# themattinthehatt/behavenet

Hardware: AMD Instinct MI355X
Metric: AE training frames/sec (128x128x1, batch 256) (higher is better)
Workload: dtype f32; 1 GPU; configs[1]: conv AE default arch, 1x128x128 f32 frames resident in HBM, 12 latents, batch 256 (chunks 200+56), fwd+bwd+Adam(amsgrad)

## Files before the change

behavenet_amd/csrc/conv_qgemm.hip:

```cpp
#include <stdlib.h>
#include "bn_common.h"
#include "bn_fast.h"

typedef float floatx16 __attribute__((ext_vector_type(16)));

#define QG_T 64
#define QG_NB 2
#define QG_KS 32
#define QG_LD 33
enum { QG_DOWN = 0, QG_UP = 1, QG_WGRAD = 2 };

struct QGArgs {
    const float* small;
    const float* big;
    const float* w;
    float* part;
    int N, Cs, Cb;
    int M, Nc, K;
    int kper;
    float* out;
    const float* bias;
    const float* dact_src;
    int act, dact;
    float slope;
};

__device__ __forceinline__ int qg_pix(int z, int j) {
    return (4 * (z >> 1) + (j >> 2)) * 8 + 4 * (z & 1) + (j & 3);
}
__device__ __forceinline__ int qg_tap(int z, int j) {
    return (((z >> 1) ? 0 : 1) + (j >> 2)) * 5 + ((z & 1) ? 0 : 1) + (j & 3);
}

typedef float floatx4a __attribute__((ext_vector_type(4)));
typedef float floatx4u __attribute__((ext_vector_type(4), aligned(4)));

template <int MODE>
__global__ __launch_bounds__(256) void k_qgemm(QGArgs a) {
    __shared__ float As[QG_T * QG_LD];
    __shared__ float Bs[QG_NB * QG_T * QG_LD];
    const int tid = threadIdx.x, lane = tid & 63;
    const int wv = __builtin_amdgcn_readfirstlane(tid >> 6);
    const int li = lane & 31, lk = lane >> 5;
    const int z = blockIdx.z & 3, ks = blockIdx.z >> 2;
    const int i0 = blockIdx.y * QG_T, j0 = blockIdx.x * (QG_NB * QG_T);
    const int kbeg = ks * a.kper;
    const int kend = min(a.K, kbeg + a.kper);
    const int zp = z >> 1, zq = z & 1;

    int ar, ak, br, bk;
    if (MODE == QG_WGRAD) { ar = tid & 63; ak = (tid >> 6) * 8; }
    else                  { ar = tid >> 2; ak = (tid & 3) * 8; }
    if (MODE == QG_DOWN)  { br = tid >> 2; bk = (tid & 3) * 8; }
    else                  { bk = tid >> 3; br = (tid & 7) * 8; }
    const bool a_ok = (i0 + ar) < a.M;

    constexpr int OOB = 0x7fffffff;
    const void* a_base = (MODE == QG_DOWN) ? (const void*)a.big : (const void*)a.small;
    const size_t a_bytes = (MODE == QG_DOWN) ? (size_t)a.N * a.Cb * 64 * 4 : (size_t)a.N * a.Cs * 4 * 4;
    const void* b_base = (MODE == QG_WGRAD) ? (const void*)a.big : (const void*)a.w;
    const size_t b_bytes = (MODE == QG_WGRAD) ? (size_t)a.N * a.Cb * 64 * 4 : (size_t)a.Cs * a.Cb * 25 * 4;
    const __amdgpu_buffer_rsrc_t rsa = __builtin_amdgcn_make_buffer_rsrc((void*)a_base, 0, (int)a_bytes, 0x00020000);
    const __amdgpu_buffer_rsrc_t rsb = __builtin_amdgcn_make_buffer_rsrc((void*)b_base, 0, (int)b_bytes, 0x00020000);
    int avo, bvo[QG_NB], a_step, b_step, a_e = 0;
    if (MODE == QG_DOWN) {
        avo = (((i0 + ar) * a.Cb + (ak >> 4)) * 64 + (4 * zp + ((ak & 15) >> 2)) * 8 + 4 * zq) * 4;
        a_step = 2 * 64 * 4;
    } else if (MODE == QG_UP) {
        avo = (z * a.N * a.Cs + (i0 + ar) * a.Cs + ak) * 4;
        a_step = QG_KS * 4;
    } else {
        avo = ((ak * a.Cs + i0 + ar) * 4 + z) * 4;
        a_e = a.Cs * 16;
        a_step = QG_KS * a.Cs * 16;
    }
    if (!a_ok) avo = OOB;
#pragma unroll
    for (int h = 0; h < QG_NB; ++h) {
        const int jc = j0 + QG_T * h + br;
        if (MODE == QG_DOWN)
            bvo[h] = ((jc * a.Cb + (bk >> 4)) * 25 + ((zp ? 0 : 1) + ((bk & 15) >> 2)) * 5 + (zq ? 0 : 1)) * 4;
        else if (MODE == QG_UP)
            bvo[h] = ((bk * a.Cb + (jc >> 4)) * 25 + ((zp ? 0 : 1) + ((jc & 15) >> 2)) * 5 + (zq ? 0 : 1)) * 4;
        else
            bvo[h] = ((bk * a.Cb + (jc >> 4)) * 64 + (4 * zp + ((jc & 15) >> 2)) * 8 + 4 * zq) * 4;
    }
    b_step = (MODE == QG_DOWN) ? 2 * 25 * 4 : (MODE == QG_UP ? QG_KS * a.Cb * 25 * 4 : QG_KS * a.Cb * 64 * 4);
    constexpr int B2ND = (MODE == QG_WGRAD) ? 32 : 20;

    float ra[8], rb[QG_NB][8];
    auto fetch = [&](const int sidx, const int k0) __attribute__((always_inline)) {
        const int sa = (MODE == QG_DOWN ? (kbeg >> 4) * 256 : (MODE == QG_UP ? kbeg * 4 : kbeg * a.Cs * 16)) + sidx * a_step;
        const int sb = (MODE == QG_DOWN ? (kbeg >> 4) * 100 : (MODE == QG_UP ? kbeg * a.Cb * 100 : kbeg * a.Cb * 256)) + sidx * b_step;
        const bool tail = (MODE == QG_WGRAD) && (k0 + QG_KS > kend);
        if (MODE == QG_WGRAD) {
#pragma unroll
            for (int e = 0; e < 8; ++e) {
                const int vo = (tail && k0 + ak + e >= kend) ? OOB : avo;
                ra[e] = __builtin_bit_cast(float, __builtin_amdgcn_raw_buffer_load_b32(rsa, vo, sa + e * a_e, 0));
            }
        } else {
            const floatx4a v0 = __builtin_bit_cast(floatx4a, __builtin_amdgcn_raw_buffer_load_b128(rsa, avo, sa, 0));
            const floatx4a v1 = __builtin_bit_cast(floatx4a, __builtin_amdgcn_raw_buffer_load_b128(
                rsa, avo, sa + (MODE == QG_DOWN ? 32 : 16), 0));
            ra[0] = v0.x; ra[1] = v0.y; ra[2] = v0.z; ra[3] = v0.w;
            ra[4] = v1.x; ra[5] = v1.y; ra[6] = v1.z; ra[7] = v1.w;
        }
#pragma unroll
        for (int h = 0; h < QG_NB; ++h) {
            const int vo = (tail && k0 + bk >= kend) ? OOB : bvo[h];
            const floatx4a w0 = __builtin_bit_cast(floatx4a, __builtin_amdgcn_raw_buffer_load_b128(rsb, vo, sb, 0));
            const floatx4a w1 = __builtin_bit_cast(floatx4a, __builtin_amdgcn_raw_buffer_load_b128(rsb, vo, sb + B2ND, 0));
            rb[h][0] = w0.x; rb[h][1] = w0.y; rb[h][2] = w0.z; rb[h][3] = w0.w;
            rb[h][4] = w1.x; rb[h][5] = w1.y; rb[h][6] = w1.z; rb[h][7] = w1.w;
        }
    };

    floatx16 acc[QG_NB];
#pragma unroll
    for (int h = 0; h < QG_NB; ++h)
#pragma unroll
        for (int t = 0; t < 16; ++t) acc[h][t] = 0.f;
    const float* ap = As + ((wv >> 1) * 32 + li) * QG_LD + lk;
    const float* bp = Bs + ((wv & 1) * 32 + li) * QG_LD + lk;

    if (kbeg < kend) fetch(0, kbeg);
    int sidx = 0;
#ifdef QG_LOOP_SHIFT
    BN_LOOP_PLACE(8, QG_LOOP_SHIFT);
#endif
    for (int k0 = kbeg; k0 < kend; k0 += QG_KS, ++sidx) {
        __syncthreads();
#pragma unroll
        for (int e = 0; e < 8; ++e) As[ar * QG_LD + ak + e] = ra[e];
#pragma unroll
        for (int h = 0; h < QG_NB; ++h)
#pragma unroll
            for (int e = 0; e < 8; ++e) {
                if (MODE == QG_DOWN) Bs[(QG_T * h + br) * QG_LD + bk + e] = rb[h][e];
                else                 Bs[(QG_T * h + br + e) * QG_LD + bk] = rb[h][e];
            }
        __syncthreads();
#pragma unroll
        for (int t = 0; t < QG_KS / 2; ++t) {
            const float av = ap[2 * t];
#pragma unroll
            for (int h = 0; h < QG_NB; ++h)
                acc[h] = __builtin_amdgcn_mfma_f32_32x32x2f32(av, bp[QG_T * h * QG_LD + 2 * t],
                                                              acc[h], 0, 0, 0);
            if (t == 1) {
                __builtin_amdgcn_sched_barrier(0);
                if (k0 + QG_KS < kend) fetch(sidx + 1, k0 + QG_KS);
                __builtin_amdgcn_sched_barrier(0);
            }
        }
    }

    if (MODE == QG_UP) {
        const int obytes = (int)((size_t)a.M * a.Cb * 64 * 4);
        const __amdgpu_buffer_rsrc_t ro = __builtin_amdgcn_make_buffer_rsrc((void*)a.out, 0, obytes, 0x00020000);
        const __amdgpu_buffer_rsrc_t rd = __builtin_amdgcn_make_buffer_rsrc(
            (void*)a.dact_src, 0, a.dact_src ? obytes : 0, 0x00020000);
        const int row_bytes = a.Cb * 64 * 4;
        const int irow = i0 + (wv >> 1) * 32 + 4 * lk;
        if (a.act != BN_ACT_SIGMOID && a.dact != BN_ACT_SIGMOID) {
            const float es = (a.act == BN_ACT_LRELU) ? a.slope : 1.f;
            const float ds = (a.dact == BN_ACT_LRELU) ? a.slope : 1.f;
#pragma unroll
            for (int h = 0; h < QG_NB; ++h) {
                const int j = j0 + QG_T * h + (wv & 1) * 32 + li;
                const int c = j >> 4;
                const float bj = a.bias ? a.bias[c] : 0.f;
                const int vo = (irow * a.Cb * 64 + c * 64 + qg_pix(z, j & 15)) * 4;
                float d[16];
                if (a.dact_src) {
#pragma unroll
                    for (int t = 0; t < 16; ++t) {
                        const int ro_t = (t & 3) + 8 * (t >> 2);
                        d[t] = __builtin_bit_cast(float, __builtin_amdgcn_raw_buffer_load_b32(
                            rd, (irow + ro_t < a.M) ? vo : 0x7fffffff, ro_t * row_bytes, 0));
                    }
                }
#pragma unroll
                for (int t = 0; t < 16; ++t) {
                    const int ro_t = (t & 3) + 8 * (t >> 2);
                    float v = acc[h][t] + bj;
                    v = v > 0.f ? v : v * es;
                    if (a.dact_src) v *= d[t] > 0.f ? 1.f : ds;
                    __builtin_amdgcn_raw_buffer_store_b32(__builtin_bit_cast(int, v), ro,
                                                          (irow + ro_t < a.M) ? vo : 0x7fffffff,
                                                          ro_t * row_bytes, 0);
                }
            }
            return;
        }
#pragma unroll
        for (int h = 0; h < QG_NB; ++h) {
            const int j = j0 + QG_T * h + (wv & 1) * 32 + li;
            const int c = j >> 4;
            const float bj = a.bias ? a.bias[c] : 0.f;
            const size_t col = (size_t)c * 64 + qg_pix(z, j & 15);
#pragma unroll
            for (int t = 0; t < 16; ++t) {
                const int i = i0 + (wv >> 1) * 32 + (t & 3) + 8 * (t >> 2) + 4 * lk;
                if (i >= a.M) continue;
                const size_t o = (size_t)i * a.Cb * 64 + col;
                float v = bn_apply_act(acc[h][t] + bj, a.act, a.slope);
                if (a.dact_src) v *= bn_act_grad_from_output(a.dact_src[o], a.dact, a.slope);
                a.out[o] = v;
            }
        }
        return;
    }
    float* dst = a.part + ((size_t)(ks * 4 + z) * a.M) * a.Nc;
#pragma unroll
    for (int h = 0; h < QG_NB; ++h) {
        const int j = j0 + QG_T * h + (wv & 1) * 32 + li;
#pragma unroll
        for (int t = 0; t < 16; ++t) {
            const int i = i0 + (wv >> 1) * 32 + (t & 3) + 8 * (t >> 2) + 4 * lk;
            if (i < a.M) dst[(size_t)i * a.Nc + j] = acc[h][t];
        }
    }
}

__global__ __launch_bounds__(256) void k_qg_split_small(const float* __restrict__ small,
                                                        float* __restrict__ dst, size_t nm) {
    const size_t idx = (size_t)blockIdx.x * 256 + threadIdx.x;
    if (idx >= nm) return;
    const floatx4a v = *reinterpret_cast<const floatx4a*>(small + 4 * idx);
    dst[idx] = v.x; dst[nm + idx] = v.y; dst[2 * nm + idx] = v.z; dst[3 * nm + idx] = v.w;
}

__global__ __launch_bounds__(256) void k_qg_finish_down(
    const float* __restrict__ part, const float* __restrict__ bias, float* __restrict__ out,
    const float* __restrict__ dact_src, int N, int Cs, int splits, int act, int dact,
    float slope) {
    const size_t total = (size_t)N * Cs * 4;
    const size_t idx = (size_t)blockIdx.x * 256 + threadIdx.x;
    if (idx >= total) return;
    const int z = (int)(idx & 3);
    const size_t nm = idx >> 2;
    const size_t plane = (size_t)N * Cs;
    float v = 0.f;
    for (int s = 0; s < splits; ++s) v += part[(size_t)(s * 4 + z) * plane + nm];
    if (bias) v += bias[nm % Cs];
    v = bn_apply_act(v, act, slope);
    if (dact_src) v *= bn_act_grad_from_output(dact_src[idx], dact, slope);
    out[idx] = v;
}

__global__ __launch_bounds__(256) void k_qg_finish_wgrad(
    const float* __restrict__ part, float* __restrict__ dw, int Cs, int Cb, int accumulate) {
    __shared__ __attribute__((aligned(16))) float stage[256 * 25];
    const size_t npair = (size_t)Cs * Cb;
    const size_t mc = (size_t)blockIdx.x * 256 + threadIdx.x;
    const size_t plane = npair * 16;
    if (mc < npair) {
        float q[4][16];
#pragma unroll
        for (int zq = 0; zq < 4; ++zq)
#pragma unroll
            for (int g4 = 0; g4 < 4; ++g4) {
                const floatx4a v = *reinterpret_cast<const floatx4a*>(part + zq * plane + mc * 16 + 4 * g4);
                q[zq][4 * g4 + 0] = v.x; q[zq][4 * g4 + 1] = v.y; q[zq][4 * g4 + 2] = v.z; q[zq][4 * g4 + 3] = v.w;
            }
#pragma unroll
        for (int tap = 0; tap < 25; ++tap) {
            const int r = tap / 5, s = tap - 5 * r;
            float v = 0.f;
#pragma unroll
            for (int p = 0; p < 2; ++p) {
                const int yy = r - (p ? 0 : 1);
                if (yy < 0 || yy > 3) continue;
#pragma unroll
                for (int qq = 0; qq < 2; ++qq) {
                    const int xx = s - (qq ? 0 : 1);
                    if (xx < 0 || xx > 3) continue;
                    v += q[2 * p + qq][4 * yy + xx];
                }
            }
            stage[threadIdx.x * 25 + tap] = v;
        }
    }
    __syncthreads();
    const size_t base = (size_t)blockIdx.x * 256 * 25;
    const size_t total = npair * 25;
    for (int i = threadIdx.x; i < 256 * 25 / 4; i += 256) {
        const size_t o = base + 4 * (size_t)i;
        if (o + 3 < total) {
            floatx4a v = *reinterpret_cast<const floatx4a*>(stage + 4 * i);
            if (accumulate) {
                const floatx4a d = *reinterpret_cast<const floatx4a*>(dw + o);
                v.x += d.x; v.y += d.y; v.z += d.z; v.w += d.w;
            }
            *reinterpret_cast<floatx4a*>(dw + o) = v;
        } else {
            for (int e = 0; e < 4; ++e)
                if (o + e < total) dw[o + e] = accumulate ? dw[o + e] + stage[4 * i + e] : stage[4 * i + e];
        }
    }
}

bool bn_qgemm_supported(const BnGeom& g) {
    if (g.R != 5 || g.S != 5 || g.stride != 5) return false;
    if (g.Hs != 2 || g.Ws != 2 || g.Hb != 8 || g.Wb != 8 || g.pt != 1 || g.pl != 1) return false;
    if ((g.Cs % (QG_NB * QG_T)) != 0 || (g.Cb % (4 * QG_NB)) != 0) return false;
    if ((size_t)g.N * g.Cb * 64 * 4 >= 0x7fffffffull) return false;
    return true;
}

static int qg_down_splits(const BnGeom& g) {
    if ((g.Cs / QG_T) * 4 >= 64) return 1;
    int s = g.Cb * 16 >= 4096 ? 4 : (g.Cb * 16 >= 2048 ? 2 : 1);
    if (g.N <= 64) {
        const int tiles = (g.Cs / (QG_NB * QG_T)) * ((g.N + QG_T - 1) / QG_T) * 4;
        while (tiles * s < 256 && s < 16 && (g.Cb * 16) / (2 * s) >= 256) s *= 2;
    }
    return s;
}

size_t bn_qgemm_ws_bytes(int role, const BnGeom& g) {
    if (role == QG_DOWN) return (size_t)qg_down_splits(g) * 4 * g.N * g.Cs * sizeof(float);
    if (role == QG_UP) return (size_t)4 * g.N * g.Cs * sizeof(float);
    return (size_t)4 * g.Cs * g.Cb * 16 * sizeof(float);
}

int bn_launch_qgemm_down(const float* big, const float* w, const float* bias, float* out,
                         const float* dact_src, const BnGeom& g, int act, int dact, float slope,
                         void* ws, hipStream_t st) {
    const int splits = qg_down_splits(g);
    QGArgs a = {nullptr, big, w, (float*)ws, g.N, g.Cs, g.Cb, g.N, g.Cs, g.Cb * 16, 0,
                nullptr, nullptr, nullptr, 0, 0, 0.f};
    a.kper = ((a.K / splits + QG_KS - 1) / QG_KS) * QG_KS;
    const dim3 grid(a.Nc / (QG_NB * QG_T), (a.M + QG_T - 1) / QG_T, 4 * splits);
    BN_LAUNCH_MAIN(k_qgemm<QG_DOWN>, grid, dim3(256), 0, st, a);
    BN_LAUNCH_CHECK();
    const size_t total = (size_t)g.N * g.Cs * 4;
    hipLaunchKernelGGL(k_qg_finish_down, dim3((unsigned)((total + 255) / 256)), dim3(256), 0, st,
                       (const float*)ws, bias, out, dact_src, g.N, g.Cs, splits, act, dact, slope);
    BN_LAUNCH_CHECK();
    return 0;
}

int bn_launch_qgemm_up(const float* small, const float* w, const float* bias, float* out,
                       const float* dact_src, const BnGeom& g, int act, int dact, float slope,
                       void* ws, hipStream_t st) {
    float* zsmall = (float*)ws;
    const size_t nm = (size_t)g.N * g.Cs;
    hipLaunchKernelGGL(k_qg_split_small, dim3((unsigned)((nm + 255) / 256)), dim3(256), 0, st, small,
                       zsmall, nm);
    BN_LAUNCH_CHECK();
    QGArgs a = {zsmall, nullptr, w, nullptr, g.N, g.Cs, g.Cb, g.N, g.Cb * 16, g.Cs, 0,
                out, bias, dact_src, act, dact, slope};
    a.kper = ((a.K + QG_KS - 1) / QG_KS) * QG_KS;
    const dim3 grid(a.Nc / (QG_NB * QG_T), (a.M + QG_T - 1) / QG_T, 4);
    BN_LAUNCH_MAIN(k_qgemm<QG_UP>, grid, dim3(256), 0, st, a);
    BN_LAUNCH_CHECK();
    return 0;
}

int bn_launch_qgemm_wgrad(const float* small, const float* big, float* dw, const BnGeom& g,
                          int accumulate, void* ws, hipStream_t st) {
    QGArgs a = {small, big, nullptr, (float*)ws, g.N, g.Cs, g.Cb, g.Cs, g.Cb * 16, g.N, 0,
                nullptr, nullptr, nullptr, 0, 0, 0.f};
    a.kper = ((a.K + QG_KS - 1) / QG_KS) * QG_KS;
    const dim3 grid(a.Nc / (QG_NB * QG_T), (a.M + QG_T - 1) / QG_T, 4);
    BN_LAUNCH_MAIN(k_qgemm<QG_WGRAD>, grid, dim3(256), 0, st, a);
    BN_LAUNCH_CHECK();
    const size_t npair = (size_t)g.Cs * g.Cb;
    hipLaunchKernelGGL(k_qg_finish_wgrad, dim3((unsigned)((npair + 255) / 256)), dim3(256), 0, st,
                       (const float*)ws, dw, g.Cs, g.Cb, accumulate);
    BN_LAUNCH_CHECK();
    return 0;
}
```

behavenet_amd/csrc/conv_qgemm2.hip:

```cpp
#include <stdlib.h>
#include "bn_common.h"
#include "bn_fast.h"

typedef float q2x16 __attribute__((ext_vector_type(16)));
typedef float q2x4 __attribute__((ext_vector_type(4)));

#define Q2_THREADS 256
#define Q2_OOB 0x7fffffff
#define Q2_MAX_LDS (160 * 1024)

__device__ __forceinline__ void q2_dma16(__amdgpu_buffer_rsrc_t rsrc, char* lds, int voffset,
                                         int soffset) {
    __builtin_amdgcn_raw_ptr_buffer_load_lds(rsrc, (float*)lds, 16, voffset, soffset, 0, 0);
}

#define Q2_R0(z) (((z) >> 1) ? 0 : 1)
#define Q2_S0(z) (((z) & 1) ? 0 : 1)

#define Q2U_KS 32
#define Q2U_PAIR 1040
#define Q2U_SBYTES (16 * Q2U_PAIR)
#define Q2U_WROW 200
#define Q2U_WINSTR 25
#define Q2U_WBYTES (Q2U_WINSTR * 1024)
#define Q2U_STAGE (Q2U_SBYTES + Q2U_WBYTES)
#define Q2U_NDMA 11

__global__ __launch_bounds__(Q2_THREADS, 1) void k_qg2_up(
    const float* __restrict__ small, const float* __restrict__ w, const float* __restrict__ bias,
    float* __restrict__ out, const float* __restrict__ dact_src, int N, int Cs, int Cb, int act,
    int dact, float slope) {
    extern __shared__ __attribute__((aligned(16))) char smem[];
    const int tid = threadIdx.x, lane = tid & 63;
    const int wv = __builtin_amdgcn_readfirstlane(tid >> 6);
    const int li = lane & 31, kh = lane >> 5;
    const int cw0 = blockIdx.x * 8, c0 = cw0 + 2 * wv, n0 = blockIdx.y * 32;

    const __amdgpu_buffer_rsrc_t rs_s = __builtin_amdgcn_make_buffer_rsrc(
        (void*)small, 0, (int)((size_t)N * Cs * 16), 0x00020000);
    const __amdgpu_buffer_rsrc_t rs_w = __builtin_amdgcn_make_buffer_rsrc(
        (void*)w, 0, (int)((size_t)Cs * Cb * 100), 0x00020000);

    const int vo_s = ((n0 + (lane >> 5)) * Cs + (lane & 31)) * 16;
    int vo_w[7];
#pragma unroll
    for (int h = 0; h < 7; ++h) {
        const int grp = 64 * (wv + 4 * h) + lane;
        const int ml = grp / 50, gi = grp - 50 * ml;
        vo_w[h] = (ml * Cb + cw0) * 100 + gi * 16;
    }
    auto issue_dma = [&](const int d, const int buf, const int stage) __attribute__((always_inline)) {
        char* base = smem + buf * Q2U_STAGE;
        if (d < 4) {
            q2_dma16(rs_s, base + (4 * wv + d) * Q2U_PAIR, vo_s, (2 * (4 * wv + d) * Cs + stage * Q2U_KS) * 16);
        } else {
            const int h = d - 4;
            if (wv + 4 * h < Q2U_WINSTR)
                q2_dma16(rs_w, base + Q2U_SBYTES + (wv + 4 * h) * 1024, vo_w[h], stage * Q2U_KS * Cb * 100);
        }
    };

    const int ad_s = (li >> 1) * Q2U_PAIR + ((li & 1) * 32 + kh) * 16;
    const int jj = li & 15;
    const int ad_w = Q2U_SBYTES + (kh * Q2U_WROW + (2 * wv + (li >> 4)) * 25 + (jj >> 2) * 5 + (jj & 3)) * 4;

    q2x16 acc[4];
#pragma unroll
    for (int z = 0; z < 4; ++z)
#pragma unroll
        for (int t = 0; t < 16; ++t) acc[z][t] = 0.f;

    const int n_stages = Cs / Q2U_KS;
#pragma unroll
    for (int d = 0; d < Q2U_NDMA; ++d) issue_dma(d, 0, 0);

#ifdef Q2U_LOOP_SHIFT
    BN_LOOP_PLACE(8, Q2U_LOOP_SHIFT);
#endif
    for (int st = 0; st < n_stages; ++st) {
        asm volatile("s_waitcnt vmcnt(0)" ::: "memory");
        __syncthreads();
        const int buf = st & 1;
#ifdef Q2_ABL_NODMA
        const bool more = false;
#else
        const bool more = st + 1 < n_stages;
#endif
        const char* sp = smem + buf * Q2U_STAGE + ad_s;
        int wo[4];
#pragma unroll
        for (int z = 0; z < 4; ++z) {
            wo[z] = buf * Q2U_STAGE + ad_w + (Q2_R0(z) * 5 + Q2_S0(z)) * 4;
            asm volatile("" : "+v"(wo[z]));
        }
        q2x4 sv[2];
        float wq[2][4];
        sv[0] = *reinterpret_cast<const q2x4*>(sp);
#pragma unroll
        for (int z = 0; z < 4; ++z) wq[0][z] = *reinterpret_cast<const float*>(smem + wo[z]);
#pragma unroll
        for (int t = 0; t < 16; ++t) {
            const int cu = t & 1, nx = cu ^ 1;
            if (t + 1 < 16) {
                sv[nx] = *reinterpret_cast<const q2x4*>(sp + (t + 1) * 32);
#pragma unroll
                for (int z = 0; z < 4; ++z)
                    wq[nx][z] = *reinterpret_cast<const float*>(smem + wo[z] + (t + 1) * 2 * Q2U_WROW * 4);
            }
            __builtin_amdgcn_sched_barrier(0);
            acc[0] = __builtin_amdgcn_mfma_f32_32x32x2f32(wq[cu][0], sv[cu].x, acc[0], 0, 0, 0);
            acc[1] = __builtin_amdgcn_mfma_f32_32x32x2f32(wq[cu][1], sv[cu].y, acc[1], 0, 0, 0);
            if (more && t < Q2U_NDMA) issue_dma(t, buf ^ 1, st + 1);
            acc[2] = __builtin_amdgcn_mfma_f32_32x32x2f32(wq[cu][2], sv[cu].z, acc[2], 0, 0, 0);
            acc[3] = __builtin_amdgcn_mfma_f32_32x32x2f32(wq[cu][3], sv[cu].w, acc[3], 0, 0, 0);
            __builtin_amdgcn_sched_barrier(0);
        }
    }

    const int n = n0 + li;
    const int obytes = (int)((size_t)N * Cb * 64 * 4);
    const __amdgpu_buffer_rsrc_t ro = __builtin_amdgcn_make_buffer_rsrc((void*)out, 0, obytes, 0x00020000);
    const __amdgpu_buffer_rsrc_t rd = __builtin_amdgcn_make_buffer_rsrc(
        (void*)dact_src, 0, dact_src ? obytes : 0, 0x00020000);
    const int vo = (n < N) ? (n * Cb + c0) * 256 : Q2_OOB;
    const float es = (act == BN_ACT_LRELU) ? slope : 1.f;
    const float ds = (dact == BN_ACT_LRELU) ? slope : 1.f;
    float bz[2] = {0.f, 0.f};
    if (bias) { bz[0] = bias[c0]; bz[1] = bias[c0 + 1]; }
#pragma unroll
    for (int z = 0; z < 4; ++z) {
        q2x4 d[4];
#pragma unroll
        for (int tq = 0; tq < 4; ++tq) {
            const int so = (tq >> 1) * 256 + ((4 * (z >> 1) + 2 * (tq & 1)) * 8 + 4 * (z & 1)) * 4;
            if (dact_src)
                d[tq] = __builtin_bit_cast(q2x4, __builtin_amdgcn_raw_buffer_load_b128(rd, vo + kh * 32, so, 0));
        }
#pragma unroll
        for (int tq = 0; tq < 4; ++tq) {
            const int so = (tq >> 1) * 256 + ((4 * (z >> 1) + 2 * (tq & 1)) * 8 + 4 * (z & 1)) * 4;
            q2x4 v;
#pragma unroll
            for (int e = 0; e < 4; ++e) {
                float x = acc[z][4 * tq + e] + bz[tq >> 1];
                x = x > 0.f ? x : x * es;
                if (dact_src) x *= d[tq][e] > 0.f ? 1.f : ds;
                v[e] = x;
            }
            __builtin_amdgcn_raw_buffer_store_b128(__builtin_bit_cast(__attribute__((ext_vector_type(4))) unsigned int, v),
                                                   ro, vo + kh * 32, so, 0);
        }
    }
}

bool bn_qg2_up_supported(const BnGeom& g, int act, int dact) {
    if (!bn_qgemm_supported(g)) return false;
    if (act == BN_ACT_SIGMOID || dact == BN_ACT_SIGMOID) return false;
    if ((g.Cs % Q2U_KS) != 0 || (g.Cb & 7) != 0) return false;
    if (((g.N + 31) / 32) * (g.Cb / 8) < 128) return false;
    return true;
}

int bn_launch_qg2_up(const float* small, const float* w, const float* bias, float* out,
                     const float* dact_src, const BnGeom& g, int act, int dact, float slope,
                     hipStream_t st) {
    static bool attr_set = false;
    if (!attr_set) {
        hipError_t e = hipFuncSetAttribute((const void*)k_qg2_up, hipFuncAttributeMaxDynamicSharedMemorySize,
                                           Q2_MAX_LDS);
        if (e != hipSuccess) return (int)e;
        attr_set = true;
    }
    const dim3 grid(g.Cb / 8, (g.N + 31) / 32);
    BN_LAUNCH_MAIN(k_qg2_up, grid, dim3(Q2_THREADS), (size_t)2 * Q2U_STAGE, st, small, w, bias, out,
                   dact_src, g.N, g.Cs, g.Cb, act, dact, slope);
    BN_LAUNCH_CHECK();
    return 0;
}

#define Q2W_KS 16
#define Q2W_SBYTES (Q2W_KS * 1024)
#define Q2W_BBYTES (Q2W_KS * 2048)
#define Q2W_STAGE (Q2W_SBYTES + Q2W_BBYTES)
#define Q2W_NBUF 3
#define Q2W_NDMA 12

__global__ __launch_bounds__(Q2_THREADS, 1) void k_qg2_wgrad(
    const float* __restrict__ small, const float* __restrict__ big, float* __restrict__ dw,
    float* __restrict__ db, int N, int Cs, int Cb, int accumulate, int bias_side) {
    extern __shared__ __attribute__((aligned(16))) char smem[];
    const int tid = threadIdx.x, lane = tid & 63;
    const int wv = __builtin_amdgcn_readfirstlane(tid >> 6);
    const int li = lane & 31, kh = lane >> 5;
    const int mb = wv & 1, cq = wv >> 1;
    const int c0 = blockIdx.x * 8, m0 = blockIdx.y * 64;

    const __amdgpu_buffer_rsrc_t rs_s = __builtin_amdgcn_make_buffer_rsrc(
        (void*)small, 0, (int)((size_t)N * Cs * 16), 0x00020000);
    const __amdgpu_buffer_rsrc_t rs_b = __builtin_amdgcn_make_buffer_rsrc(
        (void*)big, 0, (int)((size_t)N * Cb * 256), 0x00020000);
    const int vo_s = (m0 + lane) * 16;
    const int vo_b = c0 * 256 + lane * 16;
    auto issue_dma = [&](const int d, const int buf, const int stage) __attribute__((always_inline)) {
        char* base = smem + buf * Q2W_STAGE;
        if (d < 4) {
            const int nl = 4 * wv + d;
            q2_dma16(rs_s, base + nl * 1024, vo_s, (stage * Q2W_KS + nl) * Cs * 16);
        } else {
            const int nl = 4 * wv + ((d - 4) >> 1), half = (d - 4) & 1;
            q2_dma16(rs_b, base + Q2W_SBYTES + nl * 2048 + half * 1024, vo_b,
                     (stage * Q2W_KS + nl) * Cb * 256 + half * 1024);
        }
    };

    const int jj = li & 15;
    const int ad_a = (kh * 64 + 32 * mb + li) * 16;
    const int ad_b = Q2W_SBYTES + (kh * 512 + (4 * cq + (li >> 4)) * 64 + (jj >> 2) * 8 + (jj & 3)) * 4;

    q2x16 acc[2][4];
#pragma unroll
    for (int cb = 0; cb < 2; ++cb)
#pragma unroll
        for (int z = 0; z < 4; ++z)
#pragma unroll
            for (int t = 0; t < 16; ++t) acc[cb][z][t] = 0.f;
    float bsum = 0.f;
    const bool do_bias1 = (bias_side == 1) && db && blockIdx.x == 0;
    const bool do_bias2 = (bias_side == 2) && db && blockIdx.y == 0;

    const int n_stages = (N + Q2W_KS - 1) / Q2W_KS;
#pragma unroll
    for (int d = 0; d < Q2W_NDMA; ++d) issue_dma(d, 0, 0);
    if (n_stages > 1) {
#pragma unroll
        for (int d = 0; d < Q2W_NDMA; ++d) issue_dma(d, 1, 1);
    }

    int buf = 0;
#ifdef Q2W_LOOP_SHIFT
    BN_LOOP_PLACE(8, Q2W_LOOP_SHIFT);
#endif
    for (int st = 0; st < n_stages; ++st) {
        if (st + 1 < n_stages) asm volatile("s_waitcnt vmcnt(12)" ::: "memory");
        else                   asm volatile("s_waitcnt vmcnt(0)" ::: "memory");
        __builtin_amdgcn_s_barrier();
        const bool more = st + 2 < n_stages;
        const int nbuf = (buf + 2 >= Q2W_NBUF) ? buf + 2 - Q2W_NBUF : buf + 2;
        const char* base = smem + buf * Q2W_STAGE;
        if (do_bias1) {
            const char* p = base + ((tid >> 6) * 4 * 64 + (tid & 63)) * 16;
#pragma unroll
            for (int i = 0; i < 4; ++i) {
                const q2x4 v = *reinterpret_cast<const q2x4*>(p + i * 1024);
                bsum += (v.x + v.y) + (v.z + v.w);
            }
        }
        if (do_bias2) {
            const char* p = base + Q2W_SBYTES + tid * 16;
#pragma unroll
            for (int i = 0; i < 8; ++i) {
                const q2x4 v = *reinterpret_cast<const q2x4*>(p + i * 4096);
                bsum += (v.x + v.y) + (v.z + v.w);
            }
        }
        const char* ap = base + ad_a;
        int bo[4];
#pragma unroll
        for (int z = 0; z < 4; ++z) {
            bo[z] = buf * Q2W_STAGE + ad_b + (32 * (z >> 1) + 4 * (z & 1)) * 4;
            asm volatile("" : "+v"(bo[z]));
        }
        q2x4 sv[2];
        float bq[2][2][4];
        sv[0] = *reinterpret_cast<const q2x4*>(ap);
#pragma unroll
        for (int cb = 0; cb < 2; ++cb)
#pragma unroll
            for (int z = 0; z < 4; ++z) bq[0][cb][z] = *reinterpret_cast<const float*>(smem + bo[z] + cb * 512);
#pragma unroll
        for (int t = 0; t < Q2W_KS / 2; ++t) {
            const int cu = t & 1, nx = cu ^ 1;
            if (t + 1 < Q2W_KS / 2) {
                sv[nx] = *reinterpret_cast<const q2x4*>(ap + (t + 1) * 2048);
#pragma unroll
                for (int cb = 0; cb < 2; ++cb)
#pragma unroll
                    for (int z = 0; z < 4; ++z)
                        bq[nx][cb][z] = *reinterpret_cast<const float*>(smem + bo[z] + cb * 512 + (t + 1) * 4096);
            }
            __builtin_amdgcn_sched_barrier(0);
#pragma unroll
            for (int z = 0; z < 4; ++z) {
                acc[0][z] = __builtin_amdgcn_mfma_f32_32x32x2f32(sv[cu][z], bq[cu][0][z], acc[0][z], 0, 0, 0);
                acc[1][z] = __builtin_amdgcn_mfma_f32_32x32x2f32(sv[cu][z], bq[cu][1][z], acc[1][z], 0, 0, 0);
                if (more && z < 2 && t < 6) issue_dma(2 * t + z, nbuf, st + 2);
            }
            __builtin_amdgcn_sched_barrier(0);
        }
        buf = (buf + 1 >= Q2W_NBUF) ? 0 : buf + 1;
    }

    float* P = reinterpret_cast<float*>(smem);
    float* R = reinterpret_cast<float*>(smem + 4 * 32 * 128 * 4);
    float* bred = reinterpret_cast<float*>(smem + 4 * 32 * 128 * 4 + 32 * 200 * 4);
    __syncthreads();
    if (do_bias1 || do_bias2) bred[tid] = bsum;
#pragma unroll 1
    for (int h = 0; h < 2; ++h) {
        if (mb == h) {
#pragma unroll
            for (int cb = 0; cb < 2; ++cb)
#pragma unroll
                for (int z = 0; z < 4; ++z)
#pragma unroll
                    for (int t = 0; t < 16; ++t) {
                        const int m = (t & 3) + 8 * (t >> 2) + 4 * kh;
                        P[(z * 32 + m) * 128 + 64 * cq + 32 * cb + li] = acc[cb][z][t];
                    }
        }
        __syncthreads();
        {
            const int m = tid >> 3, c = tid & 7;
            float q[4][16];
#pragma unroll
            for (int z = 0; z < 4; ++z)
#pragma unroll
                for (int g4 = 0; g4 < 4; ++g4) {
                    const q2x4 v = *reinterpret_cast<const q2x4*>(P + (z * 32 + m) * 128 + c * 16 + 4 * g4);
                    q[z][4 * g4 + 0] = v.x; q[z][4 * g4 + 1] = v.y; q[z][4 * g4 + 2] = v.z; q[z][4 * g4 + 3] = v.w;
                }
#pragma unroll
            for (int tap = 0; tap < 25; ++tap) {
                const int r = tap / 5, s = tap - 5 * r;
                float v = 0.f;
#pragma unroll
                for (int zp = 0; zp < 2; ++zp) {
                    const int yy = r - (zp ? 0 : 1);
                    if (yy < 0 || yy > 3) continue;
#pragma unroll
                    for (int zq = 0; zq < 2; ++zq) {
                        const int xx = s - (zq ? 0 : 1);
                        if (xx < 0 || xx > 3) continue;
                        v += q[2 * zp + zq][4 * yy + xx];
                    }
                }
                R[m * 200 + c * 25 + tap] = v;
            }
        }
        __syncthreads();
        for (int i = tid; i < 32 * 50; i += Q2_THREADS) {
            const int m = i / 50, g4 = i - 50 * m;
            q2x4 v = *reinterpret_cast<const q2x4*>(R + m * 200 + 4 * g4);
            float* dst = dw + ((size_t)(m0 + 32 * h + m) * Cb + c0) * 25 + 4 * g4;
            if (accumulate) {
                const q2x4 d = *reinterpret_cast<const q2x4*>(dst);
                v.x += d.x; v.y += d.y; v.z += d.z; v.w += d.w;
            }
            *reinterpret_cast<q2x4*>(dst) = v;
        }
    }
    if (do_bias1 && tid < 64) {
        const float v = ((bred[tid] + bred[64 + tid]) + bred[128 + tid]) + bred[192 + tid];
        db[m0 + tid] = accumulate ? db[m0 + tid] + v : v;
    }
    if (do_bias2 && tid < 8) {
        float v = 0.f;
        for (int par = 0; par < 2; ++par)
            for (int g4 = 0; g4 < 16; ++g4) v += bred[par * 128 + tid * 16 + g4];
        db[c0 + tid] = accumulate ? db[c0 + tid] + v : v;
    }
}

bool bn_qg2_wgrad_supported(const BnGeom& g) {
    if (!bn_qgemm_supported(g)) return false;
    return (g.Cs % 64) == 0 && (g.Cb % 8) == 0;
}

int bn_launch_qg2_wgrad(const float* small, const float* big, float* dw, const BnGeom& g,
                        int accumulate, float* db, int bias_side, hipStream_t st) {
    static bool attr_set = false;
    if (!attr_set) {
        hipError_t e = hipFuncSetAttribute((const void*)k_qg2_wgrad, hipFuncAttributeMaxDynamicSharedMemorySize,
                                           Q2_MAX_LDS);
        if (e != hipSuccess) return (int)e;
        attr_set = true;
    }
    const dim3 grid(g.Cb / 8, g.Cs / 64);
    BN_LAUNCH_MAIN(k_qg2_wgrad, grid, dim3(Q2_THREADS), (size_t)Q2W_NBUF * Q2W_STAGE, st, small, big, dw,
                   db, g.N, g.Cs, g.Cb, accumulate, bias_side);
    BN_LAUNCH_CHECK();
    return 0;
}
```

Measured before the change: 58950 frames/s.

## Triple-buffer qg2 up-conv pipeline and overlap epilogue loads in wgrad

The up-conv kernel moves from double to triple buffering of its LDS stages. It waits with a partial vmcnt so two stages of DMA stay in flight, and it prefetches the dact_src tiles during the last stage's MFMAs. The wgrad kernel prefetches the existing dw values for accumulation during the final stage, defers bias summation to overlap with MFMAs, and writes both halves of the accumulator to LDS at once to drop a barrier round. It also adds optional timestamp instrumentation behind a macro, at the cost of more LDS and registers.

Result: no change. 59310 frames/s (median of 6 runs) (+0.6%).

```diff
diff --git a/behavenet_amd/csrc/conv_qgemm.hip b/behavenet_amd/csrc/conv_qgemm.hip
--- a/behavenet_amd/csrc/conv_qgemm.hip
+++ b/behavenet_amd/csrc/conv_qgemm.hip
@@ -35,6 +35,20 @@
 typedef float floatx4a __attribute__((ext_vector_type(4)));
 typedef float floatx4u __attribute__((ext_vector_type(4), aligned(4)));
 
+#ifdef BN_S5_STAMPS
+__device__ unsigned long long qg_stamps[4096][8];
+extern "C" int bn_dbg_qg_stamps(void* host, int clear) {
+    hipError_t e = hipDeviceSynchronize();
+    if (e == hipSuccess && host) e = hipMemcpyFromSymbol(host, HIP_SYMBOL(qg_stamps), sizeof(unsigned long long) * 4096 * 8);
+    if (e == hipSuccess && clear) {
+        void* p = nullptr;
+        e = hipGetSymbolAddress(&p, HIP_SYMBOL(qg_stamps));
+        if (e == hipSuccess) e = hipMemset(p, 0, sizeof(unsigned long long) * 4096 * 8);
+    }
+    return (int)e;
+}
+#endif
+
 template <int MODE>
 __global__ __launch_bounds__(256) void k_qgemm(QGArgs a) {
     __shared__ float As[QG_T * QG_LD];
@@ -47,6 +61,10 @@
     const int kbeg = ks * a.kper;
     const int kend = min(a.K, kbeg + a.kper);
     const int zp = z >> 1, zq = z & 1;
+#ifdef BN_S5_STAMPS
+    unsigned long long st_w[4] = {(unsigned long long)wall_clock64(), 0, 0, 0};
+    unsigned long long st_c[3] = {(unsigned long long)__builtin_readcyclecounter(), 0, 0}, st_t = 0;
+#endif
 
     int ar, ak, br, bk;
     if (MODE == QG_WGRAD) { ar = tid & 63; ak = (tid >> 6) * 8; }
@@ -130,6 +148,9 @@
     BN_LOOP_PLACE(8, QG_LOOP_SHIFT);
 #endif
     for (int k0 = kbeg; k0 < kend; k0 += QG_KS, ++sidx) {
+#ifdef BN_S5_STAMPS
+        st_t = __builtin_readcyclecounter();
+#endif
         __syncthreads();
 #pragma unroll
         for (int e = 0; e < 8; ++e) As[ar * QG_LD + ak + e] = ra[e];
@@ -141,6 +162,10 @@
                 else                 Bs[(QG_T * h + br + e) * QG_LD + bk] = rb[h][e];
             }
         __syncthreads();
+#ifdef BN_S5_STAMPS
+        if (sidx > 0) st_c[2] += __builtin_readcyclecounter() - st_t;
+        else st_w[1] = wall_clock64();
+#endif
 #pragma unroll
         for (int t = 0; t < QG_KS / 2; ++t) {
             const float av = ap[2 * t];
@@ -212,6 +237,9 @@
         }
         return;
     }
+#ifdef BN_S5_STAMPS
+    st_w[2] = wall_clock64();
+#endif
     float* dst = a.part + ((size_t)(ks * 4 + z) * a.M) * a.Nc;
 #pragma unroll
     for (int h = 0; h < QG_NB; ++h) {
@@ -222,6 +250,18 @@
             if (i < a.M) dst[(size_t)i * a.Nc + j] = acc[h][t];
         }
     }
+#ifdef BN_S5_STAMPS
+    if (MODE == QG_DOWN) {
+        asm volatile("s_waitcnt vmcnt(0)" ::: "memory");
+        st_w[3] = wall_clock64(); st_c[1] = __builtin_readcyclecounter();
+        const int wg = (blockIdx.z * gridDim.y + blockIdx.y) * gridDim.x + blockIdx.x;
+        if (threadIdx.x == 0 && wg < 4096) {
+            for (int i = 0; i < 4; ++i) qg_stamps[wg][i] = st_w[i];
+            for (int i = 0; i < 3; ++i) qg_stamps[wg][4 + i] = st_c[i];
+            qg_stamps[wg][7] = 1;
+        }
+    }
+#endif
 }
 
 __global__ __launch_bounds__(256) void k_qg_split_small(const float* __restrict__ small,
diff --git a/behavenet_amd/csrc/conv_qgemm2.hip b/behavenet_amd/csrc/conv_qgemm2.hip
--- a/behavenet_amd/csrc/conv_qgemm2.hip
+++ b/behavenet_amd/csrc/conv_qgemm2.hip
@@ -1,4 +1,5 @@
 #include <stdlib.h>
+#include <type_traits>
 #include "bn_common.h"
 #include "bn_fast.h"
 
@@ -13,6 +14,44 @@
                                          int soffset) {
     __builtin_amdgcn_raw_ptr_buffer_load_lds(rsrc, (float*)lds, 16, voffset, soffset, 0, 0);
 }
+
+#ifdef BN_S5_STAMPS
+__device__ unsigned long long q2_stamps[2][4096][8];
+#define Q2_STAMP_DECL unsigned long long st_w[4] = {0, 0, 0, 0}, st_c[3] = {0, 0, 0}, st_t = 0
+#define Q2_STAMP_WALL(i) st_w[i] = wall_clock64()
+#define Q2_STAMP_CYC(i) st_c[i] = __builtin_readcyclecounter()
+#define Q2_STALL_BEGIN() st_t = __builtin_readcyclecounter()
+#define Q2_STALL_END(count) do { if (count) st_c[2] += __builtin_readcyclecounter() - st_t; } while (0)
+#define Q2_STAMP_WRITE(k) do {                                                          \
+        asm volatile("s_waitcnt vmcnt(0)" ::: "memory");                                \
+        Q2_STAMP_WALL(3); Q2_STAMP_CYC(1);                                              \
+        const int wg_ = blockIdx.y * gridDim.x + blockIdx.x;                            \
+        if (threadIdx.x == 0 && wg_ < 4096) {                                           \
+            for (int i_ = 0; i_ < 4; ++i_) q2_stamps[k][wg_][i_] = st_w[i_];            \
+            for (int i_ = 0; i_ < 3; ++i_) q2_stamps[k][wg_][4 + i_] = st_c[i_];        \
+            q2_stamps[k][wg_][7] = 1;                                                   \
+        }                                                                               \
+    } while (0)
+extern "C" int bn_dbg_q2_stamps(int k, void* host, int clear) {
+    hipError_t e = hipDeviceSynchronize();
+    if (e == hipSuccess && host)
+        e = hipMemcpyFromSymbol(host, HIP_SYMBOL(q2_stamps), sizeof(unsigned long long) * 4096 * 8,
+                                sizeof(unsigned long long) * 4096 * 8 * (size_t)k);
+    if (e == hipSuccess && clear) {
+        void* p = nullptr;
+        e = hipGetSymbolAddress(&p, HIP_SYMBOL(q2_stamps));
+        if (e == hipSuccess) e = hipMemset(p, 0, sizeof(unsigned long long) * 2 * 4096 * 8);
+    }
+    return (int)e;
+}
+#else
+#define Q2_STAMP_DECL
+#define Q2_STAMP_WALL(i)
+#define Q2_STAMP_CYC(i)
+#define Q2_STALL_BEGIN()
+#define Q2_STALL_END(count)
+#define Q2_STAMP_WRITE(k)
+#endif
 
 #define Q2_R0(z) (((z) >> 1) ? 0 : 1)
 #define Q2_S0(z) (((z) & 1) ? 0 : 1)
@@ -24,6 +63,10 @@
 #define Q2U_WINSTR 25
 #define Q2U_WBYTES (Q2U_WINSTR * 1024)
 #define Q2U_STAGE (Q2U_SBYTES + Q2U_WBYTES)
+#define Q2U_NBUF 3
+#ifndef Q2U_MIN_WGS
+#define Q2U_MIN_WGS 128
+#endif
 #define Q2U_NDMA 11
 
 __global__ __launch_bounds__(Q2_THREADS, 1) void k_qg2_up(
@@ -35,6 +78,8 @@
     const int wv = __builtin_amdgcn_readfirstlane(tid >> 6);
     const int li = lane & 31, kh = lane >> 5;
     const int cw0 = blockIdx.x * 8, c0 = cw0 + 2 * wv, n0 = blockIdx.y * 32;
+    Q2_STAMP_DECL;
+    Q2_STAMP_WALL(0); Q2_STAMP_CYC(0);
 
     const __amdgpu_buffer_rsrc_t rs_s = __builtin_amdgcn_make_buffer_rsrc(
         (void*)small, 0, (int)((size_t)N * Cs * 16), 0x00020000);
@@ -71,71 +116,94 @@
         for (int t = 0; t < 16; ++t) acc[z][t] = 0.f;
 
     const int n_stages = Cs / Q2U_KS;
-#pragma unroll
-    for (int d = 0; d < Q2U_NDMA; ++d) issue_dma(d, 0, 0);
-
-#ifdef Q2U_LOOP_SHIFT
-    BN_LOOP_PLACE(8, Q2U_LOOP_SHIFT);
-#endif
-    for (int st = 0; st < n_stages; ++st) {
-        asm volatile("s_waitcnt vmcnt(0)" ::: "memory");
-        __syncthreads();
-        const int buf = st & 1;
-#ifdef Q2_ABL_NODMA
-        const bool more = false;
-#else
-        const bool more = st + 1 < n_stages;
-#endif
-        const char* sp = smem + buf * Q2U_STAGE + ad_s;
-        int wo[4];
-#pragma unroll
-        for (int z = 0; z < 4; ++z) {
-            wo[z] = buf * Q2U_STAGE + ad_w + (Q2_R0(z) * 5 + Q2_S0(z)) * 4;
-            asm volatile("" : "+v"(wo[z]));
-        }
-        q2x4 sv[2];
-        float wq[2][4];
-        sv[0] = *reinterpret_cast<const q2x4*>(sp);
-#pragma unroll
-        for (int z = 0; z < 4; ++z) wq[0][z] = *reinterpret_cast<const float*>(smem + wo[z]);
-#pragma unroll
-        for (int t = 0; t < 16; ++t) {
-            const int cu = t & 1, nx = cu ^ 1;
-            if (t + 1 < 16) {
-                sv[nx] = *reinterpret_cast<const q2x4*>(sp + (t + 1) * 32);
-#pragma unroll
-                for (int z = 0; z < 4; ++z)
-                    wq[nx][z] = *reinterpret_cast<const float*>(smem + wo[z] + (t + 1) * 2 * Q2U_WROW * 4);
-            }
-            __builtin_amdgcn_sched_barrier(0);
-            acc[0] = __builtin_amdgcn_mfma_f32_32x32x2f32(wq[cu][0], sv[cu].x, acc[0], 0, 0, 0);
-            acc[1] = __builtin_amdgcn_mfma_f32_32x32x2f32(wq[cu][1], sv[cu].y, acc[1], 0, 0, 0);
-            if (more && t < Q2U_NDMA) issue_dma(t, buf ^ 1, st + 1);
-            acc[2] = __builtin_amdgcn_mfma_f32_32x32x2f32(wq[cu][2], sv[cu].z, acc[2], 0, 0, 0);
-            acc[3] = __builtin_amdgcn_mfma_f32_32x32x2f32(wq[cu][3], sv[cu].w, acc[3], 0, 0, 0);
-            __builtin_amdgcn_sched_barrier(0);
-        }
-    }
 
     const int n = n0 + li;
     const int obytes = (int)((size_t)N * Cb * 64 * 4);
     const __amdgpu_buffer_rsrc_t ro = __builtin_amdgcn_make_buffer_rsrc((void*)out, 0, obytes, 0x00020000);
     const __amdgpu_buffer_rsrc_t rd = __builtin_amdgcn_make_buffer_rsrc(
         (void*)dact_src, 0, dact_src ? obytes : 0, 0x00020000);
-    const int vo = (n < N) ? (n * Cb + c0) * 256 : Q2_OOB;
+    const int vo = ((n < N) ? (n * Cb + c0) * 256 : Q2_OOB) + ((n < N) ? kh * 32 : 0);
     const float es = (act == BN_ACT_LRELU) ? slope : 1.f;
     const float ds = (dact == BN_ACT_LRELU) ? slope : 1.f;
     float bz[2] = {0.f, 0.f};
     if (bias) { bz[0] = bias[c0]; bz[1] = bias[c0 + 1]; }
+    q2x4 dsrc[16];
+
+    auto stage = [&](auto last_c, const int buf, const int nbuf, const int st) __attribute__((always_inline)) {
+        constexpr bool LAST = decltype(last_c)::value;
+#ifdef Q2_ABL_NODMA
+        const bool more = false;
+#else
+        const bool more = !LAST && st + 2 < n_stages;
+#endif
+        const char* sp = smem + buf * Q2U_STAGE + ad_s;
+        int wo[4];
+#pragma unroll
+        for (int z = 0; z < 4; ++z) {
+            wo[z] = buf * Q2U_STAGE + ad_w + (Q2_R0(z) * 5 + Q2_S0(z)) * 4;
+            asm volatile("" : "+v"(wo[z]));
+        }
+        q2x4 sv[2];
+        float wq[2][4];
+        sv[0] = *reinterpret_cast<const q2x4*>(sp);
+#pragma unroll
+        for (int z = 0; z < 4; ++z) wq[0][z] = *reinterpret_cast<const float*>(smem + wo[z]);
+#pragma unroll
+        for (int t = 0; t < 16; ++t) {
+            const int cu = t & 1, nx = cu ^ 1;
+            if (t + 1 < 16) {
+                sv[nx] = *reinterpret_cast<const q2x4*>(sp + (t + 1) * 32);
+#pragma unroll
+                for (int z = 0; z < 4; ++z)
+                    wq[nx][z] = *reinterpret_cast<const float*>(smem + wo[z] + (t + 1) * 2 * Q2U_WROW * 4);
+            }
+            __builtin_amdgcn_sched_barrier(0);
+            acc[0] = __builtin_amdgcn_mfma_f32_32x32x2f32(wq[cu][0], sv[cu].x, acc[0], 0, 0, 0);
+            acc[1] = __builtin_amdgcn_mfma_f32_32x32x2f32(wq[cu][1], sv[cu].y, acc[1], 0, 0, 0);
+            if (!LAST) {
+                if (more && t < Q2U_NDMA) issue_dma(t, nbuf, st + 2);
+            } else if (dact_src) {
+                const int z = t >> 2, tq = t & 3;
+                const int so = (tq >> 1) * 256 + ((4 * (z >> 1) + 2 * (tq & 1)) * 8 + 4 * (z & 1)) * 4;
+                dsrc[t] = __builtin_bit_cast(q2x4, __builtin_amdgcn_raw_buffer_load_b128(rd, vo, so, 0));
+            }
+            acc[2] = __builtin_amdgcn_mfma_f32_32x32x2f32(wq[cu][2], sv[cu].z, acc[2], 0, 0, 0);
+            acc[3] = __builtin_amdgcn_mfma_f32_32x32x2f32(wq[cu][3], sv[cu].w, acc[3], 0, 0, 0);
+            __builtin_amdgcn_sched_barrier(0);
+        }
+    };
+
+#pragma unroll
+    for (int d = 0; d < Q2U_NDMA; ++d) issue_dma(d, 0, 0);
+    if (n_stages > 1) {
+#pragma unroll
+        for (int d = 0; d < Q2U_NDMA; ++d) issue_dma(d, 1, 1);
+    }
+
+    int buf = 0;
+#ifdef Q2U_LOOP_SHIFT
+    BN_LOOP_PLACE(8, Q2U_LOOP_SHIFT);
+#endif
+    for (int st = 0; st + 1 < n_stages; ++st) {
+        Q2_STALL_BEGIN();
+        asm volatile("s_waitcnt vmcnt(10)" ::: "memory");
+        __builtin_amdgcn_s_barrier();
+        Q2_STALL_END(st > 0);
+        if (st == 0) { Q2_STAMP_WALL(1); }
+        const int nbuf = (buf + 2 >= Q2U_NBUF) ? buf + 2 - Q2U_NBUF : buf + 2;
+        stage(std::false_type(), buf, nbuf, st);
+        buf = (buf + 1 >= Q2U_NBUF) ? 0 : buf + 1;
+    }
+    Q2_STALL_BEGIN();
+    asm volatile("s_waitcnt vmcnt(0)" ::: "memory");
+    __builtin_amdgcn_s_barrier();
+    Q2_STALL_END(n_stages > 1);
+    if (n_stages == 1) { Q2_STAMP_WALL(1); }
+    stage(std::true_type(), buf, 0, n_stages - 1);
+
+    Q2_STAMP_WALL(2);
 #pragma unroll
     for (int z = 0; z < 4; ++z) {
-        q2x4 d[4];
-#pragma unroll
-        for (int tq = 0; tq < 4; ++tq) {
-            const int so = (tq >> 1) * 256 + ((4 * (z >> 1) + 2 * (tq & 1)) * 8 + 4 * (z & 1)) * 4;
-            if (dact_src)
-                d[tq] = __builtin_bit_cast(q2x4, __builtin_amdgcn_raw_buffer_load_b128(rd, vo + kh * 32, so, 0));
-        }
 #pragma unroll
         for (int tq = 0; tq < 4; ++tq) {
             const int so = (tq >> 1) * 256 + ((4 * (z >> 1) + 2 * (tq & 1)) * 8 + 4 * (z & 1)) * 4;
@@ -144,20 +212,21 @@
             for (int e = 0; e < 4; ++e) {
                 float x = acc[z][4 * tq + e] + bz[tq >> 1];
                 x = x > 0.f ? x : x * es;
-                if (dact_src) x *= d[tq][e] > 0.f ? 1.f : ds;
+                if (dact_src) x *= dsrc[4 * z + tq][e] > 0.f ? 1.f : ds;
                 v[e] = x;
             }
             __builtin_amdgcn_raw_buffer_store_b128(__builtin_bit_cast(__attribute__((ext_vector_type(4))) unsigned int, v),
-                                                   ro, vo + kh * 32, so, 0);
-        }
-    }
+                                                   ro, vo, so, 0);
+        }
+    }
+    Q2_STAMP_WRITE(0);
 }
 
 bool bn_qg2_up_supported(const BnGeom& g, int act, int dact) {
     if (!bn_qgemm_supported(g)) return false;
     if (act == BN_ACT_SIGMOID || dact == BN_ACT_SIGMOID) return false;
     if ((g.Cs % Q2U_KS) != 0 || (g.Cb & 7) != 0) return false;
-    if (((g.N + 31) / 32) * (g.Cb / 8) < 128) return false;
+    if (((g.N + 31) / 32) * (g.Cb / 8) < Q2U_MIN_WGS) return false;
     return true;
 }
 
@@ -172,7 +241,7 @@
         attr_set = true;
     }
     const dim3 grid(g.Cb / 8, (g.N + 31) / 32);
-    BN_LAUNCH_MAIN(k_qg2_up, grid, dim3(Q2_THREADS), (size_t)2 * Q2U_STAGE, st, small, w, bias, out,
+    BN_LAUNCH_MAIN(k_qg2_up, grid, dim3(Q2_THREADS), (size_t)Q2U_NBUF * Q2U_STAGE, st, small, w, bias, out,
                    dact_src, g.N, g.Cs, g.Cb, act, dact, slope);
     BN_LAUNCH_CHECK();
     return 0;
@@ -183,6 +252,9 @@
 #define Q2W_BBYTES (Q2W_KS * 2048)
 #define Q2W_STAGE (Q2W_SBYTES + Q2W_BBYTES)
 #define Q2W_NBUF 3
+#define Q2W_PBYTES (2 * 4 * 32 * 128 * 4)
+#define Q2W_RBYTES (32 * 200 * 4)
+#define Q2W_LDS (Q2W_PBYTES + Q2W_RBYTES + 1024)
 #define Q2W_NDMA 12
 
 __global__ __launch_bounds__(Q2_THREADS, 1) void k_qg2_wgrad(
@@ -194,6 +266,8 @@
     const int li = lane & 31, kh = lane >> 5;
     const int mb = wv & 1, cq = wv >> 1;
     const int c0 = blockIdx.x * 8, m0 = blockIdx.y * 64;
+    Q2_STAMP_DECL;
+    Q2_STAMP_WALL(0); Q2_STAMP_CYC(0);
 
     const __amdgpu_buffer_rsrc_t rs_s = __builtin_amdgcn_make_buffer_rsrc(
         (void*)small, 0, (int)((size_t)N * Cs * 16), 0x00020000);
@@ -236,32 +310,42 @@
         for (int d = 0; d < Q2W_NDMA; ++d) issue_dma(d, 1, 1);
     }
 
+    const __amdgpu_buffer_rsrc_t rs_d = __builtin_amdgcn_make_buffer_rsrc(
+        (void*)dw, 0, (int)((size_t)Cs * Cb * 100), 0x00020000);
+    int vo_d[7];
+#pragma unroll
+    for (int j = 0; j < 7; ++j) {
+        const int i = tid + Q2_THREADS * j;
+        const int m = i / 50, g4 = i - 50 * m;
+        vo_d[j] = (i < 32 * 50) ? (m * Cb * 25 + 4 * g4) * 4 : Q2_OOB;
+    }
+    q2x4 dpre[14];
+
     int buf = 0;
 #ifdef Q2W_LOOP_SHIFT
     BN_LOOP_PLACE(8, Q2W_LOOP_SHIFT);
 #endif
     for (int st = 0; st < n_stages; ++st) {
+        Q2_STALL_BEGIN();
         if (st + 1 < n_stages) asm volatile("s_waitcnt vmcnt(12)" ::: "memory");
         else                   asm volatile("s_waitcnt vmcnt(0)" ::: "memory");
         __builtin_amdgcn_s_barrier();
+        Q2_STALL_END(st > 0);
+        if (st == 0) { Q2_STAMP_WALL(1); }
         const bool more = st + 2 < n_stages;
+        const bool pre = accumulate && st + 1 == n_stages;
         const int nbuf = (buf + 2 >= Q2W_NBUF) ? buf + 2 - Q2W_NBUF : buf + 2;
         const char* base = smem + buf * Q2W_STAGE;
+        q2x4 bv[8];
         if (do_bias1) {
             const char* p = base + ((tid >> 6) * 4 * 64 + (tid & 63)) * 16;
 #pragma unroll
-            for (int i = 0; i < 4; ++i) {
-                const q2x4 v = *reinterpret_cast<const q2x4*>(p + i * 1024);
-                bsum += (v.x + v.y) + (v.z + v.w);
-            }
+            for (int i = 0; i < 4; ++i) bv[i] = *reinterpret_cast<const q2x4*>(p + i * 1024);
         }
         if (do_bias2) {
             const char* p = base + Q2W_SBYTES + tid * 16;
 #pragma unroll
-            for (int i = 0; i < 8; ++i) {
-                const q2x4 v = *reinterpret_cast<const q2x4*>(p + i * 4096);
-                bsum += (v.x + v.y) + (v.z + v.w);
-            }
+            for (int i = 0; i < 8; ++i) bv[i] = *reinterpret_cast<const q2x4*>(p + i * 4096);
         }
         const char* ap = base + ad_a;
         int bo[4];
@@ -294,31 +378,45 @@
                 acc[0][z] = __builtin_amdgcn_mfma_f32_32x32x2f32(sv[cu][z], bq[cu][0][z], acc[0][z], 0, 0, 0);
                 acc[1][z] = __builtin_amdgcn_mfma_f32_32x32x2f32(sv[cu][z], bq[cu][1][z], acc[1][z], 0, 0, 0);
                 if (more && z < 2 && t < 6) issue_dma(2 * t + z, nbuf, st + 2);
+                if (pre && z >= 2 && t < 7) {
+                    const int q = 2 * t + z - 2;
+                    dpre[q] = __builtin_bit_cast(q2x4, __builtin_amdgcn_raw_buffer_load_b128(
+                        rs_d, vo_d[q % 7], ((m0 + 32 * (q / 7)) * Cb + c0) * 100, 0));
+                }
+            }
+            if (t == 1) {
+                if (do_bias1) {
+#pragma unroll
+                    for (int i = 0; i < 4; ++i) bsum += (bv[i].x + bv[i].y) + (bv[i].z + bv[i].w);
+                }
+                if (do_bias2) {
+#pragma unroll
+                    for (int i = 0; i < 8; ++i) bsum += (bv[i].x + bv[i].y) + (bv[i].z + bv[i].w);
+                }
             }
             __builtin_amdgcn_sched_barrier(0);
         }
         buf = (buf + 1 >= Q2W_NBUF) ? 0 : buf + 1;
     }
 
+    Q2_STAMP_WALL(2);
     float* P = reinterpret_cast<float*>(smem);
-    float* R = reinterpret_cast<float*>(smem + 4 * 32 * 128 * 4);
-    float* bred = reinterpret_cast<float*>(smem + 4 * 32 * 128 * 4 + 32 * 200 * 4);
+    float* bred = reinterpret_cast<float*>(smem + Q2W_PBYTES + Q2W_RBYTES);
     __syncthreads();
     if (do_bias1 || do_bias2) bred[tid] = bsum;
-#pragma unroll 1
+#pragma unroll
+    for (int cb = 0; cb < 2; ++cb)
+#pragma unroll
+        for (int z = 0; z < 4; ++z)
+#pragma unroll
+            for (int t = 0; t < 16; ++t) {
+                const int m = (t & 3) + 8 * (t >> 2) + 4 * kh;
+                P[((mb * 4 + z) * 32 + m) * 128 + 64 * cq + 32 * cb + li] = acc[cb][z][t];
+            }
+    __syncthreads();
+#pragma unroll
     for (int h = 0; h < 2; ++h) {
-        if (mb == h) {
-#pragma unroll
-            for (int cb = 0; cb < 2; ++cb)
-#pragma unroll
-                for (int z = 0; z < 4; ++z)
-#pragma unroll
-                    for (int t = 0; t < 16; ++t) {
-                        const int m = (t & 3) + 8 * (t >> 2) + 4 * kh;
-                        P[(z * 32 + m) * 128 + 64 * cq + 32 * cb + li] = acc[cb][z][t];
-                    }
-        }
-        __syncthreads();
+        float* R = reinterpret_cast<float*>(smem + (h ? 0 : Q2W_PBYTES));
         {
             const int m = tid >> 3, c = tid & 7;
             float q[4][16];
@@ -326,7 +424,7 @@
             for (int z = 0; z < 4; ++z)
 #pragma unroll
                 for (int g4 = 0; g4 < 4; ++g4) {
-                    const q2x4 v = *reinterpret_cast<const q2x4*>(P + (z * 32 + m) * 128 + c * 16 + 4 * g4);
+                    const q2x4 v = *reinterpret_cast<const q2x4*>(P + ((h * 4 + z) * 32 + m) * 128 + c * 16 + 4 * g4);
                     q[z][4 * g4 + 0] = v.x; q[z][4 * g4 + 1] = v.y; q[z][4 * g4 + 2] = v.z; q[z][4 * g4 + 3] = v.w;
                 }
 #pragma unroll
@@ -348,15 +446,19 @@
             }
         }
         __syncthreads();
-        for (int i = tid; i < 32 * 50; i += Q2_THREADS) {
-            const int m = i / 50, g4 = i - 50 * m;
-            q2x4 v = *reinterpret_cast<const q2x4*>(R + m * 200 + 4 * g4);
-            float* dst = dw + ((size_t)(m0 + 32 * h + m) * Cb + c0) * 25 + 4 * g4;
-            if (accumulate) {
-                const q2x4 d = *reinterpret_cast<const q2x4*>(dst);
-                v.x += d.x; v.y += d.y; v.z += d.z; v.w += d.w;
-            }
-            *reinterpret_cast<q2x4*>(dst) = v;
+#pragma unroll
+        for (int j = 0; j < 7; ++j) {
+            const int i = tid + Q2_THREADS * j;
+            if (i < 32 * 50) {
+                const int m = i / 50, g4 = i - 50 * m;
+                q2x4 v = *reinterpret_cast<const q2x4*>(R + m * 200 + 4 * g4);
+                float* dst = dw + ((size_t)(m0 + 32 * h + m) * Cb + c0) * 25 + 4 * g4;
+                if (accumulate) {
+                    const q2x4 d = dpre[7 * h + j];
+                    v.x += d.x; v.y += d.y; v.z += d.z; v.w += d.w;
+                }
+                *reinterpret_cast<q2x4*>(dst) = v;
+            }
         }
     }
     if (do_bias1 && tid < 64) {
@@ -369,12 +471,16 @@
             for (int g4 = 0; g4 < 16; ++g4) v += bred[par * 128 + tid * 16 + g4];
         db[c0 + tid] = accumulate ? db[c0 + tid] + v : v;
     }
+    Q2_STAMP_WRITE(1);
 }
 
 bool bn_qg2_wgrad_supported(const BnGeom& g) {
     if (!bn_qgemm_supported(g)) return false;
     return (g.Cs % 64) == 0 && (g.Cb % 8) == 0;
 }
+
+static_assert(Q2W_LDS >= Q2W_NBUF * Q2W_STAGE && Q2W_LDS <= Q2_MAX_LDS, "k_qg2_wgrad LDS");
+static_assert(Q2U_NBUF * Q2U_STAGE <= Q2_MAX_LDS, "k_qg2_up LDS");
 
 int bn_launch_qg2_wgrad(const float* small, const float* big, float* dw, const BnGeom& g,
                         int accumulate, float* db, int bias_side, hipStream_t st) {
@@ -386,7 +492,7 @@
         attr_set = true;
     }
     const dim3 grid(g.Cb / 8, g.Cs / 64);
-    BN_LAUNCH_MAIN(k_qg2_wgrad, grid, dim3(Q2_THREADS), (size_t)Q2W_NBUF * Q2W_STAGE, st, small, big, dw,
+    BN_LAUNCH_MAIN(k_qg2_wgrad, grid, dim3(Q2_THREADS), (size_t)Q2W_LDS, st, small, big, dw,
                    db, g.N, g.Cs, g.Cb, accumulate, bias_side);
     BN_LAUNCH_CHECK();
     return 0;
```
